# JuliaGaussianProcesses/Stheno.jl

Measured on AMD Instinct MI355X. Metric: logpdf_per_sec, higher is better.
Workload: dtype f64; 1 GPU; single GP, matern52, N=65536, D=8, lengthscale sqrt(D), sigma2=0.1 (BASELINE config 'c5'); N=65536, D=8, kernel=matern52, parallelism=1 GPU

## Files before the change

### stheno.jl_amd/csrc/gemm_nt.hip

```cpp
#include "common.h"
#include "potrf_diag.h"
#include "tilemap.h"
#include "kstep.h"

namespace sgp {

constexpr int KB = 16;

__device__ __forceinline__ bool tile_of_block(long n_tr, long n_tc, long mask_off, long& tr, long& tc) {
  return tile_of_id((long)blockIdx.x, n_tr, n_tc, mask_off, tr, tc);
}

template <bool HANDOFF, bool STAMP = false>
__device__ __forceinline__ bool gemm_nt_dma_tile(const double* A, long lda, const double* B, long ldb, double* C,
                                                 long ldc, long K, double alpha, double beta, long mask_off,
                                                 long n_tr, long n_tc, long c_slice_stride, const double* Cin,
                                                 long ldcin, int klo, double* smem, long& tr, long& tc,
                                                 long long* dbg = nullptr, const TileSkip* sk = nullptr,
                                                 bool keep_first = false) {
  long long st0 = 0, st1 = 0, st2 = 0, stA = 0;
  if (STAMP) st0 = (long long)__builtin_amdgcn_s_memtime();
  constexpr int NJ = 8, WCOLS = 32;
  if (klo == 3) {
    const long sub = mask_off > 1 ? mask_off : 1;
    const long tiles = n_tr * (n_tr + 1) / 2, full = sub > 1 ? tiles / 64 * 64 : tiles;
    const long sl = (long)blockIdx.x & 7;
    long k = (long)blockIdx.x >> 3, q = 0, kk = K;
    if (k >= full) {
      const long e = k - full;
      k = full + e / sub;
      q = e % sub;
      kk = K / sub;
    }
    tr = (long)((sqrt(8.0 * (double)k + 1.0) - 1.0) * 0.5);
    while (tr * (tr + 1) / 2 > k) --tr;
    while ((tr + 1) * (tr + 2) / 2 <= k) ++tr;
    tc = k - tr * (tr + 1) / 2;
    if (tr >= n_tr) return false;
    A += (sl * K + q * kk) * lda;
    B += (sl * K + q * kk) * ldb;
    C += (sl * sub + q) * c_slice_stride;
    K = kk;
  } else {
    if (sk && sk->cmap) {
      const int x = (int)(blockIdx.x & 7), pos = (int)(blockIdx.x >> 3);
      if (pos >= sk->cmap[x]) return false;
      if (!tile_of_id((long)sk->cmap[16 + (long)x * sk->cstride + pos] * 8 + x, n_tr, n_tc, mask_off, tr, tc)) return false;
    } else if (!tile_of_block(n_tr, n_tc, mask_off, tr, tc)) return false;
    A += (long)blockIdx.y * K * lda;
    B += (long)blockIdx.y * K * ldb;
    C += (long)blockIdx.y * c_slice_stride;
  }
  if (sk && sk->nz) {
    if (sk->need0 >= 0) {
      const sz_word* rn = sk->nz + (long)(sk->need0 + tr) * sk->words;
      if (!((rn[tc >> 6] >> (tc & 63)) & 1)) return false;
    }
    const sz_word* ra = sk->nz + (long)(sk->tr0 + tr) * sk->words;
    const sz_word* rb = sk->nz + (long)(sk->tc0 + tc) * sk->words;
    int kmin = -1, kmax = -1;
    for (int q = sk->kt0 >> 6; q <= (sk->kt1 - 1) >> 6; ++q) {
      sz_word m = ra[q] & rb[q];
      if (q == (sk->kt0 >> 6)) m &= ~(sz_word)0 << (sk->kt0 & 63);
      if (q == ((sk->kt1 - 1) >> 6) && (sk->kt1 & 63)) m &= ~(~(sz_word)0 << (sk->kt1 & 63));
      if (m != 0) {
        if (kmin < 0) kmin = q * 64 + (int)__builtin_ctzll(m);
        kmax = q * 64 + 63 - (int)__builtin_clzll(m);
      }
    }
    if (kmin < 0) {
      if (sk->need0 >= 0)
        K = 0;
      else if (!(keep_first && tr == 0 && tc == 0))
        return false;
    } else {
      A += (long)(kmin - sk->kt0) * TILE * lda;
      B += (long)(kmin - sk->kt0) * TILE * ldb;
      K = (long)(kmax - kmin + 1) * TILE;
    }
  }
  if (STAMP) stA = (long long)__builtin_amdgcn_s_memtime();
  const int t = threadIdx.x;
  const int lane = t & 63;
  const int w = t >> 6;
  const int wr = w >> 2, wc = w & 3;
  const int l15 = lane & 15, lq = lane >> 4, l3 = lane & 3;
  const double* Ag = A + tr * TILE;
  const double* Bg = B + tc * TILE;
  double* Cg = C + (tr * TILE + wr * 64 + l15) + (tc * TILE + wc * WCOLS + lq) * ldc;
  const double* Cs = Cin + (tr * TILE + wr * 64 + l15) + (tc * TILE + wc * WCOLS + lq) * ldcin;
  double acc[NJ][4];
  typedef const __attribute__((address_space(1))) void* gptr_t;
  typedef __attribute__((address_space(3))) void* lptr_t;
  const int wu = __builtin_amdgcn_readfirstlane(w);
  const unsigned lds_base = (unsigned)(unsigned long long)(__attribute__((address_space(3))) double*)smem;
  auto dma = [&](long k0, int stage) {
    double* sa = smem + stage * (2 * KB * LDS_LD);
    double* sb = sa + KB * LDS_LD;
#pragma unroll
    for (int i = 0; i < KB / 8; ++i) {
      const int col = wu + 8 * i;
      __builtin_amdgcn_global_load_lds((gptr_t)(Ag + 2 * lane + (k0 + col) * lda), (lptr_t)(sa + col * LDS_LD), 16, 0, 0);
      __builtin_amdgcn_global_load_lds((gptr_t)(Bg + 2 * lane + (k0 + col) * ldb), (lptr_t)(sb + col * LDS_LD), 16, 0, 0);
    }
  };
  long nchunks = K / KB;
  const long cbeg = klo == 1 ? tr * (TILE / KB) : 0;
  if (klo == 2 && (tr + 1) * (TILE / KB) < nchunks) nchunks = (tr + 1) * (TILE / KB);
  auto kof = [&](long c) { return c * KB; };
  if (cbeg < nchunks) dma(kof(cbeg), 0);
  if (beta != 0.0) {
#pragma unroll
    for (int j = 0; j < NJ; ++j)
#pragma unroll
      for (int i = 0; i < 4; ++i) acc[j][i] = Cs[i * 16 + (long)(j * 4) * ldcin];
    const double seed = beta / alpha;
#pragma unroll
    for (int j = 0; j < NJ; ++j)
#pragma unroll
      for (int i = 0; i < 4; ++i) acc[j][i] *= seed;
  } else {
#pragma unroll
    for (int j = 0; j < NJ; ++j)
#pragma unroll
      for (int i = 0; i < 4; ++i) acc[j][i] = 0.0;
  }
  asm volatile("s_waitcnt vmcnt(0)" ::: "memory");
  __builtin_amdgcn_s_barrier();
  if (STAMP) st1 = (long long)__builtin_amdgcn_s_memtime();
  for (long c = cbeg; c < nchunks; ++c) {
    const int stage = (int)(c & 1);
    if (c + 1 < nchunks) dma(kof(c + 1), stage ^ 1);
    const unsigned a_addr = lds_base + (unsigned)((stage * (2 * KB * LDS_LD) + lq * LDS_LD + wr * 64 + l15) * 8);
    const unsigned b_addr = lds_base + (unsigned)((stage * (2 * KB * LDS_LD) + KB * LDS_LD + lq * LDS_LD + wc * WCOLS + l3) * 8);
    {
      double a_r[4], b_c[NJ];
      asm volatile("ds_read_b64 %0, %1 offset:0" : "=v"(a_r[0]) : "v"(a_addr));
      asm volatile("ds_read_b64 %0, %1 offset:128" : "=v"(a_r[1]) : "v"(a_addr));
      asm volatile("ds_read_b64 %0, %1 offset:256" : "=v"(a_r[2]) : "v"(a_addr));
      asm volatile("ds_read_b64 %0, %1 offset:384" : "=v"(a_r[3]) : "v"(a_addr));
      asm volatile("ds_read_b64 %0, %1 offset:0" : "=v"(b_c[0]) : "v"(b_addr));
      asm volatile("ds_read_b64 %0, %1 offset:32" : "=v"(b_c[1]) : "v"(b_addr));
      asm volatile("ds_read_b64 %0, %1 offset:64" : "=v"(b_c[2]) : "v"(b_addr));
      asm volatile("ds_read_b64 %0, %1 offset:96" : "=v"(b_c[3]) : "v"(b_addr));
      asm volatile("ds_read_b64 %0, %1 offset:128" : "=v"(b_c[4]) : "v"(b_addr));
      asm volatile("ds_read_b64 %0, %1 offset:160" : "=v"(b_c[5]) : "v"(b_addr));
      asm volatile("ds_read_b64 %0, %1 offset:192" : "=v"(b_c[6]) : "v"(b_addr));
      asm volatile("ds_read_b64 %0, %1 offset:224" : "=v"(b_c[7]) : "v"(b_addr));
      asm volatile("s_waitcnt lgkmcnt(0)" ::: "memory");
      __builtin_amdgcn_sched_barrier(0);
#pragma unroll
      for (int j = 0; j < NJ; ++j)
#pragma unroll
        for (int i = 0; i < 4; ++i) acc[j][i] = mfma44_f64(b_c[j], a_r[i], acc[j][i]);
    }
    {
      double a_r[4], b_c[NJ];
      asm volatile("ds_read_b64 %0, %1 offset:4608" : "=v"(a_r[0]) : "v"(a_addr));
      asm volatile("ds_read_b64 %0, %1 offset:4736" : "=v"(a_r[1]) : "v"(a_addr));
      asm volatile("ds_read_b64 %0, %1 offset:4864" : "=v"(a_r[2]) : "v"(a_addr));
      asm volatile("ds_read_b64 %0, %1 offset:4992" : "=v"(a_r[3]) : "v"(a_addr));
      asm volatile("ds_read_b64 %0, %1 offset:4608" : "=v"(b_c[0]) : "v"(b_addr));
      asm volatile("ds_read_b64 %0, %1 offset:4640" : "=v"(b_c[1]) : "v"(b_addr));
      asm volatile("ds_read_b64 %0, %1 offset:4672" : "=v"(b_c[2]) : "v"(b_addr));
      asm volatile("ds_read_b64 %0, %1 offset:4704" : "=v"(b_c[3]) : "v"(b_addr));
      asm volatile("ds_read_b64 %0, %1 offset:4736" : "=v"(b_c[4]) : "v"(b_addr));
      asm volatile("ds_read_b64 %0, %1 offset:4768" : "=v"(b_c[5]) : "v"(b_addr));
      asm volatile("ds_read_b64 %0, %1 offset:4800" : "=v"(b_c[6]) : "v"(b_addr));
      asm volatile("ds_read_b64 %0, %1 offset:4832" : "=v"(b_c[7]) : "v"(b_addr));
      asm volatile("s_waitcnt lgkmcnt(0)" ::: "memory");
      __builtin_amdgcn_sched_barrier(0);
#pragma unroll
      for (int j = 0; j < NJ; ++j)
#pragma unroll
        for (int i = 0; i < 4; ++i) acc[j][i] = mfma44_f64(b_c[j], a_r[i], acc[j][i]);
    }
    {
      double a_r[4], b_c[NJ];
      asm volatile("ds_read_b64 %0, %1 offset:9216" : "=v"(a_r[0]) : "v"(a_addr));
      asm volatile("ds_read_b64 %0, %1 offset:9344" : "=v"(a_r[1]) : "v"(a_addr));
      asm volatile("ds_read_b64 %0, %1 offset:9472" : "=v"(a_r[2]) : "v"(a_addr));
      asm volatile("ds_read_b64 %0, %1 offset:9600" : "=v"(a_r[3]) : "v"(a_addr));
      asm volatile("ds_read_b64 %0, %1 offset:9216" : "=v"(b_c[0]) : "v"(b_addr));
      asm volatile("ds_read_b64 %0, %1 offset:9248" : "=v"(b_c[1]) : "v"(b_addr));
      asm volatile("ds_read_b64 %0, %1 offset:9280" : "=v"(b_c[2]) : "v"(b_addr));
      asm volatile("ds_read_b64 %0, %1 offset:9312" : "=v"(b_c[3]) : "v"(b_addr));
      asm volatile("ds_read_b64 %0, %1 offset:9344" : "=v"(b_c[4]) : "v"(b_addr));
      asm volatile("ds_read_b64 %0, %1 offset:9376" : "=v"(b_c[5]) : "v"(b_addr));
      asm volatile("ds_read_b64 %0, %1 offset:9408" : "=v"(b_c[6]) : "v"(b_addr));
      asm volatile("ds_read_b64 %0, %1 offset:9440" : "=v"(b_c[7]) : "v"(b_addr));
      asm volatile("s_waitcnt lgkmcnt(0)" ::: "memory");
      __builtin_amdgcn_sched_barrier(0);
#pragma unroll
      for (int j = 0; j < NJ; ++j)
#pragma unroll
        for (int i = 0; i < 4; ++i) acc[j][i] = mfma44_f64(b_c[j], a_r[i], acc[j][i]);
    }
    {
      double a_r[4], b_c[NJ];
      asm volatile("ds_read_b64 %0, %1 offset:13824" : "=v"(a_r[0]) : "v"(a_addr));
      asm volatile("ds_read_b64 %0, %1 offset:13952" : "=v"(a_r[1]) : "v"(a_addr));
      asm volatile("ds_read_b64 %0, %1 offset:14080" : "=v"(a_r[2]) : "v"(a_addr));
      asm volatile("ds_read_b64 %0, %1 offset:14208" : "=v"(a_r[3]) : "v"(a_addr));
      asm volatile("ds_read_b64 %0, %1 offset:13824" : "=v"(b_c[0]) : "v"(b_addr));
      asm volatile("ds_read_b64 %0, %1 offset:13856" : "=v"(b_c[1]) : "v"(b_addr));
      asm volatile("ds_read_b64 %0, %1 offset:13888" : "=v"(b_c[2]) : "v"(b_addr));
      asm volatile("ds_read_b64 %0, %1 offset:13920" : "=v"(b_c[3]) : "v"(b_addr));
      asm volatile("ds_read_b64 %0, %1 offset:13952" : "=v"(b_c[4]) : "v"(b_addr));
      asm volatile("ds_read_b64 %0, %1 offset:13984" : "=v"(b_c[5]) : "v"(b_addr));
      asm volatile("ds_read_b64 %0, %1 offset:14016" : "=v"(b_c[6]) : "v"(b_addr));
      asm volatile("ds_read_b64 %0, %1 offset:14048" : "=v"(b_c[7]) : "v"(b_addr));
      asm volatile("s_waitcnt lgkmcnt(0)" ::: "memory");
      __builtin_amdgcn_sched_barrier(0);
#pragma unroll
      for (int j = 0; j < NJ; ++j)
#pragma unroll
        for (int i = 0; i < 4; ++i) acc[j][i] = mfma44_f64(b_c[j], a_r[i], acc[j][i]);
    }
    asm volatile("s_waitcnt vmcnt(0) lgkmcnt(0)" ::: "memory");
    __builtin_amdgcn_s_barrier();
  }
  if (STAMP) st2 = (long long)__builtin_amdgcn_s_memtime();
  if (HANDOFF && tr == 0 && tc == 0) {
#pragma unroll
    for (int j = 0; j < NJ; ++j)
#pragma unroll
      for (int i = 0; i < 4; ++i) {
        const int rb = 4 * wr + i, cb = 2 * wc + (j >> 2);
        const int k = 4 * (j & 3) + lq;
        if (rb >= cb) smem[boff(rb, cb) + k * 16 + l15] = (rb > cb || l15 >= k) ? alpha * acc[j][i] : 0.0;
      }
    return true;
  }
#pragma unroll
  for (int j = 0; j < NJ; ++j)
#pragma unroll
    for (int i = 0; i < 4; ++i) Cg[i * 16 + (long)(j * 4) * ldc] = alpha * acc[j][i];
  if (STAMP) {
    asm volatile("s_waitcnt vmcnt(0)" ::: "memory");
    if (threadIdx.x == 0) {
      long long* d = dbg + (long)blockIdx.x * 8;
      d[0] = st0;
      d[1] = st1;
      d[2] = st2;
      d[3] = (long long)__builtin_amdgcn_s_memtime();
      d[4] = (long long)((__builtin_amdgcn_s_getreg(6164) & 15) << 16 | (__builtin_amdgcn_s_getreg(63492) & 0xffff));
      d[5] = tr;
      d[6] = tc;
      d[7] = stA;
    }
  }
  return true;
}

__global__ __launch_bounds__(512, 4) void gemm_nt_dma_stamp_kernel(const double* A, long lda, double* C, long ldc, long K,
                                                                   long n_tr, long n_tc, long long* dbg) {
  __shared__ __attribute__((aligned(16))) double smem[2 * 2 * KB * LDS_LD];
  long tr, tc;
  gemm_nt_dma_tile<false, true>(A, lda, A, lda, C, ldc, K, -1.0, 1.0, 0L, n_tr, n_tc, 0L, C, ldc, 0, smem, tr, tc, dbg);
}

int launch_gemm_nt_stamps(const double* P, long ldp, double* C, long ldc, long M, long Nc, long K, long long* dbg,
                          long* n_ids, hipStream_t s) {
  long n_tr = M / TILE, n_tc = Nc / TILE;
  long per_xcd = tri_ids_per_xcd(tri_shape(n_tr, n_tc, -1));
  *n_ids = per_xcd * 8;
  if (!dbg) return 0;
  hipLaunchKernelGGL(gemm_nt_dma_stamp_kernel, dim3((unsigned)(per_xcd * 8)), dim3(512), 0, s, P, ldp, C, ldc, K, n_tr, n_tc, dbg);
  SGP_HIP(hipGetLastError());
  return 0;
}

template <int TAG>
__global__ __launch_bounds__(512, 4) void gemm_nt_dma_kernel(const double* A, long lda,
                                                             const double* B, long ldb, double* C,
                                                             long ldc, long K, double alpha,
                                                             double beta, long mask_off, long n_tr,
                                                             long n_tc, long c_slice_stride,
                                                             const double* Cin, long ldcin, int klo, TileSkip sk) {
  __shared__ __attribute__((aligned(16))) double smem[2 * 2 * KB * LDS_LD];
  long tr, tc;
  gemm_nt_dma_tile<false>(A, lda, B, ldb, C, ldc, K, alpha, beta, mask_off, n_tr, n_tc, c_slice_stride, Cin, ldcin,
                          klo, smem, tr, tc, nullptr, &sk);
}

template <int TAG, bool HANDOFF>
__global__ __launch_bounds__(512, 4) void gemm_nt_dma_potrf_kernel(const double* A, long lda, const double* B,
                                                                   long ldb, double* C, long ldc, long K,
                                                                   long n_tr, long n_tc, double* invd,
                                                                   double* logdet_slot, int* info, long gcol0,
                                                                   int prio, TileSkip sk) {
  extern __shared__ __attribute__((aligned(16))) double dyn_smem[];
  long tr, tc;
  const bool live = gemm_nt_dma_tile<HANDOFF>(A, lda, B, ldb, C, ldc, K, -1.0, 1.0, 0L, n_tr, n_tc, 0L, C, ldc, 0,
                                              dyn_smem, tr, tc, nullptr, &sk, true);
  if (live && tr == 0 && tc == 0) {
    if (!HANDOFF) {
      __threadfence_block();
    }
    __syncthreads();
    potrf_diag_body<false, double, HANDOFF>(C, ldc, invd, logdet_slot, info, gcol0, prio, nullptr);
  }
}

__global__ __launch_bounds__(512, 4) void gemm_nt_seg_kernel(SegBatch b) {
  __shared__ __attribute__((aligned(16))) double smem[2 * 2 * KB * LDS_LD];
  unsigned id = blockIdx.x;
  if (b.cmap) {
    const int x = (int)(id & 7), pos = (int)(id >> 3);
    if (pos >= b.cmap[x]) return;
    id = (unsigned)b.cmap[16 + (long)x * b.cstride + pos] * 8u + (unsigned)x;
  }
  int d = 0;
  for (int q = 1; q < b.n_dst; ++q)
    if (id >= b.dst[q].id0) d = q;
  d = __builtin_amdgcn_readfirstlane(d);
  const long c0 = b.dst[d].c0;
  const long n_tr = (b.m_tot - c0) / TILE, n_tc = b.dst[d].w / TILE;
  long tr, tc;
  if (!tile_of_id((long)(id - b.dst[d].id0), n_tr, n_tc, 0L, tr, tc)) return;
  const int t = threadIdx.x;
  const int lane = t & 63;
  const int w = t >> 6;
  const int wu = __builtin_amdgcn_readfirstlane(w);
  const int wr = w >> 2, wc = w & 3;
  const int l15 = lane & 15, lq = lane >> 4, l3 = lane & 3;
  const long ldc = b.dst[d].ldc;
  double* Cg = b.dst[d].C + (tr * TILE + wr * 64 + l15) + (tc * TILE + wc * 32 + lq) * ldc;
  typedef const __attribute__((address_space(1))) void* gptr_t;
  typedef __attribute__((address_space(3))) void* lptr_t;
  const unsigned lds_base = (unsigned)(unsigned long long)(__attribute__((address_space(3))) double*)smem;
  int s = b.dst[d].s_first;
  const int s_end = s + b.dst[d].s_count;
  const sz_word* ra = b.nz ? b.nz + (c0 / TILE + tr) * b.nz_words : nullptr;
  const sz_word* rb = b.nz ? b.nz + (c0 / TILE + tc) * b.nz_words : nullptr;
  auto range_of = [&](int q, int& first, int& count) {
    first = 0;
    count = b.src[q].w / KB;
    if (!ra) return;
    const long kc = b.src[q].k0 >= 0 ? b.src[q].k0 : b.src[q].row0;
    const int kt0 = (int)(kc / TILE), kt1 = (int)((kc + b.src[q].w + TILE - 1) / TILE);
    int kmin = -1, kmax = -1;
    for (int k = kt0; k < kt1; ++k)
      if ((((ra[k >> 6] & rb[k >> 6]) >> (k & 63)) & 1) != 0) {
        if (kmin < 0) kmin = k;
        kmax = k;
      }
    if (kmin < 0) {
      count = -1;
    } else if (kc % TILE == 0 && b.src[q].w % TILE == 0) {
      first = (kmin - kt0) * (TILE / KB);
      count = (kmax - kmin + 1) * (TILE / KB);
    }
  };
  unsigned livemask = ~0u;
  long total = 0;
  {
    livemask = 0;
    for (int q = s; q < s_end; ++q) {
      int f, cnt;
      range_of(q, f, cnt);
      if (cnt > 0) {
        livemask |= 1u << q;
        total += cnt;
      }
    }
    if (livemask == 0) return;
    while (!((livemask >> s) & 1)) ++s;
  }
  const double *pa = nullptr, *pb = nullptr;
  long ld = 0;
  int left = 0;
  auto open = [&](int q) {
    const long r0 = c0 - b.src[q].row0;
    ld = b.src[q].ld;
    int f, cnt;
    range_of(q, f, cnt);
    const long skip = (long)f * KB * ld;
    pa = b.src[q].base + r0 + tr * TILE + skip;
    pb = b.src[q].base + r0 + tc * TILE + skip;
    left = cnt;
  };
  auto request = [&](int stage) {
    double* sa = smem + stage * (2 * KB * LDS_LD);
    double* sb = sa + KB * LDS_LD;
#pragma unroll
    for (int i = 0; i < KB / 8; ++i) {
      const int col = wu + 8 * i;
      __builtin_amdgcn_global_load_lds((gptr_t)(pa + 2 * lane + col * ld), (lptr_t)(sa + col * LDS_LD), 16, 0, 0);
      __builtin_amdgcn_global_load_lds((gptr_t)(pb + 2 * lane + col * ld), (lptr_t)(sb + col * LDS_LD), 16, 0, 0);
    }
    pa += KB * ld;
    pb += KB * ld;
    if (--left == 0) {
      ++s;
      while (s < s_end && !((livemask >> s) & 1)) ++s;
      if (s < s_end) open(s);
    }
  };
  double acc[8][4];
  if (total > 0) {
    open(s);
    request(0);
  }
#pragma unroll
  for (int j = 0; j < 8; ++j)
#pragma unroll
    for (int i = 0; i < 4; ++i) acc[j][i] = Cg[i * 16 + (long)(j * 4) * ldc];
#pragma unroll
  for (int j = 0; j < 8; ++j)
#pragma unroll
    for (int i = 0; i < 4; ++i) acc[j][i] *= -1.0;
  asm volatile("s_waitcnt vmcnt(0)" ::: "memory");
  __builtin_amdgcn_s_barrier();
  const unsigned a_off = (unsigned)((lq * LDS_LD + wr * 64 + l15) * 8);
  const unsigned b_off = (unsigned)((KB * LDS_LD + lq * LDS_LD + wc * 32 + l3) * 8);
  for (long c = 0; c < total; ++c) {
    const int stage = (int)(c & 1);
    if (c + 1 < total) request(stage ^ 1);
    const unsigned a_addr = lds_base + (unsigned)(stage * (2 * KB * LDS_LD) * 8) + a_off;
    const unsigned b_addr = lds_base + (unsigned)(stage * (2 * KB * LDS_LD) * 8) + b_off;
    tile_kstep<0>(acc, a_addr, b_addr);
    tile_kstep<1>(acc, a_addr, b_addr);
    tile_kstep<2>(acc, a_addr, b_addr);
    tile_kstep<3>(acc, a_addr, b_addr);
    asm volatile("s_waitcnt vmcnt(0) lgkmcnt(0)" ::: "memory");
    __builtin_amdgcn_s_barrier();
  }
#pragma unroll
  for (int j = 0; j < 8; ++j)
#pragma unroll
    for (int i = 0; i < 4; ++i) Cg[i * 16 + (long)(j * 4) * ldc] = -acc[j][i];
}

__global__ __launch_bounds__(1024) void seg_compact_kernel(SegBatch b, int per_xcd, int* out) {
  __shared__ int s_wave[16];
  __shared__ int s_base;
  const int x = blockIdx.x, t = threadIdx.x, lane = t & 63, w = t >> 6;
  if (t == 0) s_base = 0;
  __syncthreads();
  for (int k0 = 0; k0 < per_xcd; k0 += 1024) {
    const int k = k0 + t;
    bool live = false;
    if (k < per_xcd) {
      const unsigned id = (unsigned)k * 8u + (unsigned)x;
      int d = 0;
      for (int q = 1; q < b.n_dst; ++q)
        if (id >= b.dst[q].id0) d = q;
      const long c0 = b.dst[d].c0;
      long tr, tc;
      if (tile_of_id((long)(id - b.dst[d].id0), (b.m_tot - c0) / TILE, b.dst[d].w / TILE, 0L, tr, tc)) {
        const sz_word* ra = b.nz + (c0 / TILE + tr) * b.nz_words;
        const sz_word* rb = b.nz + (c0 / TILE + tc) * b.nz_words;
        for (int q = b.dst[d].s_first; q < b.dst[d].s_first + b.dst[d].s_count && !live; ++q) {
          const long kc = b.src[q].k0 >= 0 ? b.src[q].k0 : b.src[q].row0;
          const int kt0 = (int)(kc / TILE), kt1 = (int)((kc + b.src[q].w + TILE - 1) / TILE);
          for (int kk = kt0; kk < kt1 && !live; ++kk) live = (((ra[kk >> 6] & rb[kk >> 6]) >> (kk & 63)) & 1) != 0;
        }
      }
    }
    const unsigned long long bal = __ballot(live);
    const int pre = __popcll(bal & ((1ull << lane) - 1ull));
    if (lane == 0) s_wave[w] = __popcll(bal);
    __syncthreads();
    int woff = 0, tot = 0;
    for (int q = 0; q < 16; ++q) {
      if (q < w) woff += s_wave[q];
      tot += s_wave[q];
    }
    const int base = s_base;
    if (live) out[16 + (long)x * per_xcd + base + woff + pre] = k;
    __syncthreads();
    if (t == 0) s_base = base + tot;
    __syncthreads();
  }
  if (t == 0) out[x] = s_base;
}

int launch_gemm_nt_seg(SegBatch& b, hipStream_t s, long* n_ids) {
  if (b.n_dst <= 0) return 0;
  if (b.n_dst > SEG_MAX_DST || b.m_tot % TILE) {
    set_error("gemm_nt_seg: bad batch");
    return -1;
  }
  long ids = 0;
  for (int d = 0; d < b.n_dst; ++d) {
    const SegDst& D = b.dst[d];
    if (D.c0 % TILE || D.w % TILE || D.w <= 0 || D.c0 + D.w > b.m_tot || D.s_first < 0 || D.s_count < 0 ||
        D.s_first + D.s_count > SEG_MAX_SRC) {
      set_error("gemm_nt_seg: bad destination panel");
      return -1;
    }
    for (int q = D.s_first; q < D.s_first + D.s_count; ++q)
      if (b.src[q].w % KB || b.src[q].w <= 0 || b.src[q].row0 > D.c0) {
        set_error("gemm_nt_seg: bad source panel");
        return -1;
      }
    b.dst[d].id0 = (unsigned)ids;
    ids += tile_ids((b.m_tot - D.c0) / TILE, D.w / TILE, 0);
  }
  if (ids >= (1L << 31)) {
    set_error("gemm_nt_seg: too many tiles for one launch");
    return -1;
  }
  if (n_ids) *n_ids = ids;
  const int* map = nullptr;
  if (b.nz && b.map_scratch && ids >= b.map_min_ids && 16 + ids <= b.map_ints) {
    b.cmap = nullptr;
    hipLaunchKernelGGL(seg_compact_kernel, dim3(8), dim3(1024), 0, s, b, (int)(ids / 8), b.map_scratch);
    SGP_HIP(hipGetLastError());
    map = b.map_scratch;
  }
  b.cmap = map;
  b.cstride = (int)(ids / 8);
  hipLaunchKernelGGL(gemm_nt_seg_kernel, dim3((unsigned)ids), dim3(512), 0, s, b);
  SGP_HIP(hipGetLastError());
  return 0;
}

#define SGP_COMPUTE(buf_, NJ_, COL0_)                                            \
  {                                                                              \
    const double* pa = &sA[buf_][wr * 64 + l15];                                 \
    const double* pb = &sB[buf_][(COL0_) + l3];                                  \
    _Pragma("unroll") for (int ks = 0; ks < 4; ++ks) {                           \
      const int kk = ks * 4 + lq;                                                \
      double a_r[4], b_c[NJ_];                                                   \
      _Pragma("unroll") for (int i = 0; i < 4; ++i) a_r[i] = pa[kk * LDS_LD + i * 16]; \
      _Pragma("unroll") for (int j = 0; j < NJ_; ++j) b_c[j] = pb[kk * LDS_LD + j * 4]; \
      _Pragma("unroll") for (int j = 0; j < NJ_; ++j)                            \
          _Pragma("unroll") for (int i = 0; i < 4; ++i)                          \
              acc[j][i] = mfma44_f64(b_c[j], a_r[i], acc[j][i]);                 \
    }                                                                            \
  }

template <bool KCAP>
__global__ __launch_bounds__(512, 4) void gemm_nt_reg_kernel(const double* A, long lda,
                                                             const double* B, long ldb, double* C,
                                                             long ldc, long K, double alpha,
                                                             double beta, long mask_off,
                                                             long kcap_off, long n_tr, long n_tc) {
  constexpr int NJ = 8, WCOLS = 32, NU = 2;
  long tr, tc;
  if (!tile_of_block(n_tr, n_tc, mask_off, tr, tc)) return;
  long Keff = K;
  if (KCAP) {
    long cap = (tc + 1) * TILE + kcap_off;
    if (cap < Keff) Keff = cap;
    if (Keff <= 0) Keff = 0;
  }
  __shared__ __attribute__((aligned(16))) double sA[2][KB * LDS_LD];
  __shared__ __attribute__((aligned(16))) double sB[2][KB * LDS_LD];
  const int t = threadIdx.x;
  const int lane = t & 63;
  const int w = t >> 6;
  const int wr = w >> 2, wc = w & 3;
  const int l15 = lane & 15, lq = lane >> 4, l3 = lane & 3;
  const double* Ag = A + tr * TILE;
  const double* Bg = B + tc * TILE;
  const int scol = t >> 6;
  const int srow = 2 * (t & 63);
  double2 ra[NU], rb[NU];
  double* Cg = C + (tr * TILE + wr * 64 + l15) + (tc * TILE + wc * WCOLS + lq) * ldc;
  double acc[NJ][4];
  if (beta != 0.0) {
    const double seed = beta / alpha;
#pragma unroll
    for (int j = 0; j < NJ; ++j)
#pragma unroll
      for (int i = 0; i < 4; ++i) acc[j][i] = Cg[i * 16 + (long)(j * 4) * ldc];
#pragma unroll
    for (int j = 0; j < NJ; ++j)
#pragma unroll
      for (int i = 0; i < 4; ++i) acc[j][i] *= seed;
  } else {
#pragma unroll
    for (int j = 0; j < NJ; ++j)
#pragma unroll
      for (int i = 0; i < 4; ++i) acc[j][i] = 0.0;
  }
#define SGP_GLOAD(k0_)                                                           \
  _Pragma("unroll") for (int i = 0; i < NU; ++i) {                               \
    long col = (k0_) + scol + 8 * i;                                             \
    ra[i] = *reinterpret_cast<const double2*>(Ag + srow + col * lda);            \
    rb[i] = *reinterpret_cast<const double2*>(Bg + srow + col * ldb);            \
  }
#define SGP_SSTORE(buf_)                                                         \
  _Pragma("unroll") for (int i = 0; i < NU; ++i) {                               \
    int col = scol + 8 * i;                                                      \
    *reinterpret_cast<double2*>(&sA[buf_][col * LDS_LD + srow]) = ra[i];         \
    *reinterpret_cast<double2*>(&sB[buf_][col * LDS_LD + srow]) = rb[i];         \
  }
  if (Keff > 0) {
    SGP_GLOAD(0);
    SGP_SSTORE(0);
    __syncthreads();
    int buf = 0;
    for (long k0 = KB; k0 < Keff; k0 += KB) {
      SGP_GLOAD(k0);
      SGP_COMPUTE(buf, NJ, wc * WCOLS);
      SGP_SSTORE(buf ^ 1);
      __syncthreads();
      buf ^= 1;
    }
    SGP_COMPUTE(buf, NJ, wc * WCOLS);
  }
#undef SGP_GLOAD
#undef SGP_SSTORE
#pragma unroll
  for (int j = 0; j < NJ; ++j)
#pragma unroll
    for (int i = 0; i < 4; ++i) Cg[i * 16 + (long)(j * 4) * ldc] = alpha * acc[j][i];
}

namespace {
struct GemmStructure {
  const char* base = nullptr;
  long elem = 8;
  long ld = 0;
  const sz_word* nz = nullptr;
  int words = 0;
  int* scratch = nullptr;
  long scratch_ints = 0;
  long tile0 = 0;
  long ncols = 0;
  hipStream_t stream2 = nullptr;
  int* scratch2 = nullptr;
};
thread_local GemmStructure g_st;
TileSkip skip_for_bytes(const void* P, long ldp, const void* C, long ldc, long K, long elem) {
  TileSkip sk;
  if (!g_st.nz || ldp != g_st.ld || ldc != g_st.ld || elem != g_st.elem) return sk;
  const long oc = ((const char*)C - g_st.base) / elem, op = ((const char*)P - g_st.base) / elem;
  if ((const char*)C < g_st.base || (const char*)P < g_st.base || oc >= g_st.ld * g_st.ncols || op >= g_st.ld * g_st.ncols) return sk;
  const long cr = oc % g_st.ld, cc = oc / g_st.ld, pr = op % g_st.ld, pc = op / g_st.ld;
  if (cr != cc || pr != cr || cr % TILE || pc % TILE || K % TILE || pc + K > cc) return sk;
  sk.nz = g_st.nz;
  sk.words = g_st.words;
  sk.tr0 = sk.tc0 = (int)(cr / TILE + g_st.tile0);
  sk.kt0 = (int)(pc / TILE + g_st.tile0);
  sk.kt1 = sk.kt0 + (int)(K / TILE);
  return sk;
}
TileSkip skip_for(const double* P, long ldp, const double* C, long ldc, long K) { return skip_for_bytes(P, ldp, C, ldc, K, 8); }
StripSkip strip_skip_bytes(const void* X, long ldx, long elem) {
  StripSkip sk;
  if (!g_st.nz || ldx != g_st.ld || elem != g_st.elem || (const char*)X < g_st.base) return sk;
  const long ox = ((const char*)X - g_st.base) / elem;
  if (ox >= g_st.ld * g_st.ncols) return sk;
  const long xr = ox % g_st.ld, xc = ox / g_st.ld;
  if (xr % TILE || xc % TILE || xr <= xc) return sk;
  sk.nz = g_st.nz;
  sk.words = g_st.words;
  sk.tr0 = (int)(xr / TILE + g_st.tile0);
  sk.kt = (int)(xc / TILE + g_st.tile0);
  return sk;
}
}
void gemm_set_structure(const double* base, long ld, const sz_word* d_nz, int words, long ncols, int* scratch,
                        long scratch_ints, long tile0, hipStream_t stream2, int* scratch2) {
  g_st.base = (const char*)base;
  g_st.elem = 8;
  g_st.ld = ld;
  g_st.nz = d_nz;
  g_st.words = words;
  g_st.scratch = scratch;
  g_st.scratch_ints = scratch_ints;
  g_st.tile0 = tile0;
  g_st.ncols = ncols;
  g_st.stream2 = stream2;
  g_st.scratch2 = scratch2;
}
void gemm_set_structure_f32(const float* base, long ld, const sz_word* d_nz, int words, long ncols) {
  gemm_set_structure(nullptr, ld, d_nz, words, ncols);
  g_st.base = (const char*)base;
  g_st.elem = 4;
}
TileSkip gemm_skip_for_f32(const float* P, long ldp, const float* C, long ldc, long K) { return skip_for_bytes(P, ldp, C, ldc, K, 4); }
StripSkip strip_skip_for_f32(const float* X, long ldx) { return strip_skip_bytes(X, ldx, 4); }
StripSkip strip_skip_for(const double* X, long ldx) { return strip_skip_bytes(X, ldx, 8); }

__global__ __launch_bounds__(1024) void tile_compact_kernel(TileSkip sk, long n_tr, long n_tc, int per_xcd, int* out,
                                                            int keep_first) {
  __shared__ int s_wave[16];
  __shared__ int s_base;
  const int x = blockIdx.x, t = threadIdx.x, lane = t & 63, w = t >> 6;
  if (t == 0) s_base = 0;
  __syncthreads();
  for (int k0 = 0; k0 < per_xcd; k0 += 1024) {
    const int k = k0 + t;
    bool live = false;
    long tr, tc;
    if (k < per_xcd && tile_of_id((long)k * 8 + x, n_tr, n_tc, 0L, tr, tc)) {
      const sz_word* ra = sk.nz + (long)(sk.tr0 + tr) * sk.words;
      const sz_word* rb = sk.nz + (long)(sk.tc0 + tc) * sk.words;
      for (int q = sk.kt0 >> 6; q <= (sk.kt1 - 1) >> 6; ++q) {
        sz_word m = ra[q] & rb[q];
        if (q == (sk.kt0 >> 6)) m &= ~(sz_word)0 << (sk.kt0 & 63);
        if (q == ((sk.kt1 - 1) >> 6) && (sk.kt1 & 63)) m &= ~(~(sz_word)0 << (sk.kt1 & 63));
        live = live || m != 0;
      }
      live = live || (keep_first && tr == 0 && tc == 0);
    }
    const unsigned long long bal = __ballot(live);
    const int pre = __popcll(bal & ((1ull << lane) - 1ull));
    if (lane == 0) s_wave[w] = __popcll(bal);
    __syncthreads();
    int woff = 0, tot = 0;
    for (int q = 0; q < 16; ++q) {
      if (q < w) woff += s_wave[q];
      tot += s_wave[q];
    }
    const int base = s_base;
    if (live) out[16 + (long)x * per_xcd + base + woff + pre] = k;
    __syncthreads();
    if (t == 0) s_base = base + tot;
    __syncthreads();
  }
  if (t == 0) out[x] = s_base;
}
static int maybe_compact(TileSkip& sk, long n_tr, long n_tc, long per_xcd, int keep_first, hipStream_t s) {
  int* map = (g_st.scratch2 && s == g_st.stream2) ? g_st.scratch2 : g_st.scratch;
  if (!sk.nz || !map || per_xcd * 8 < 4096 || 16 + per_xcd * 8 > g_st.scratch_ints) return 0;
  hipLaunchKernelGGL(tile_compact_kernel, dim3(8), dim3(1024), 0, s, sk, n_tr, n_tc, (int)per_xcd, map, keep_first);
  SGP_HIP(hipGetLastError());
  sk.cmap = map;
  sk.cstride = (int)per_xcd;
  return 0;
}

int launch_gemm_nt(const double* A, long lda, const double* B, long ldb, double* C, long ldc,
                   long M, long Nc, long K, double alpha, double beta, long mask_off,
                   int kcap_mode, long kcap_off, hipStream_t s) {
  constexpr long REG_BASELINE = -(1L << 50);
  if (M <= 0 || Nc <= 0) return 0;
  if (M % TILE || Nc % TILE || K % KB) {
    set_error("gemm_nt: M, Nc must be multiples of 128 and K of 16");
    return -1;
  }
  long n_tr = M / TILE, n_tc = Nc / TILE;
  long groups = ((n_tr + 7) / 8 + 7) / 8;
  long per_xcd = (mask_off == 0) ? tri_ids_per_xcd(tri_shape(n_tr, n_tc, -1)) : groups * 8 * n_tc;
  dim3 grid((unsigned)(per_xcd * 8));
  if (kcap_mode)
    hipLaunchKernelGGL((gemm_nt_reg_kernel<true>), grid, dim3(512), 0, s, A, lda, B, ldb, C, ldc, K, alpha,
                       beta, mask_off, kcap_off, n_tr, n_tc);
  else if (kcap_off == REG_BASELINE)
    hipLaunchKernelGGL((gemm_nt_reg_kernel<false>), grid, dim3(512), 0, s, A, lda, B, ldb, C, ldc, K, alpha,
                       beta, mask_off, 0L, n_tr, n_tc);
  else
    hipLaunchKernelGGL(gemm_nt_dma_kernel<0>, grid, dim3(512), 0, s, A, lda, B, ldb, C, ldc, K, alpha, beta,
                       mask_off, n_tr, n_tc, 0L, (const double*)C, ldc, 0,
                       (A == B && mask_off == 0 && alpha == -1.0 && beta == 1.0) ? skip_for(A, lda, C, ldc, K) : TileSkip());
  SGP_HIP(hipGetLastError());
  return 0;
}

int launch_gemm_nt_update(const double* P, long ldp, double* C, long ldc, long M, long Nc, long K, hipStream_t s) {
  if (M <= 0 || Nc <= 0) return 0;
  if (M % TILE || Nc % TILE || K % KB) {
    set_error("gemm_nt_update: M, Nc must be multiples of 128 and K of 16");
    return -1;
  }
  long n_tr = M / TILE, n_tc = Nc / TILE;
  long per_xcd = tri_ids_per_xcd(tri_shape(n_tr, n_tc, -1));
  TileSkip sk = skip_for(P, ldp, C, ldc, K);
  if (int rc = maybe_compact(sk, n_tr, n_tc, per_xcd, 0, s)) return rc;
  hipLaunchKernelGGL(gemm_nt_dma_kernel<1>, dim3((unsigned)(per_xcd * 8)), dim3(512), 0, s, P, ldp, P, ldp, C, ldc, K,
                     -1.0, 1.0, 0L, n_tr, n_tc, 0L, (const double*)C, ldc, 0, sk);
  SGP_HIP(hipGetLastError());
  return 0;
}

template <int TAG, bool HANDOFF>
static int launch_potrf_variant(unsigned grid, const double* P, long ldp, double* C, long ldc, long K, long n_tr,
                                long n_tc, double* d_invd, double* d_logdet_slot, int* d_info, long gcol0,
                                hipStream_t s) {
  SGP_LDS_ATTR_ONCE((gemm_nt_dma_potrf_kernel<TAG, HANDOFF>), PD_LDS);
  TileSkip sk = skip_for(P, ldp, C, ldc, K);
  if (int rc = maybe_compact(sk, n_tr, n_tc, (long)grid / 8, 1, s)) return rc;
  hipLaunchKernelGGL((gemm_nt_dma_potrf_kernel<TAG, HANDOFF>), dim3(grid), dim3(512), PD_LDS, s, P, ldp, P, ldp, C, ldc,
                     K, n_tr, n_tc, d_invd, d_logdet_slot, d_info, gcol0, panel_prio(), sk);
  SGP_HIP(hipGetLastError());
  return 0;
}

int launch_gemm_nt_potrf(const double* P, long ldp, double* C, long ldc, long M, long Nc, long K, int outer,
                         int handoff, double* d_invd, double* d_logdet_slot, int* d_info, long gcol0,
                         hipStream_t s) {
  if (M <= 0 || Nc <= 0) return 0;
  if (M % TILE || Nc % TILE || K % KB) {
    set_error("gemm_nt_potrf: M, Nc must be multiples of 128 and K of 16");
    return -1;
  }
  long n_tr = M / TILE, n_tc = Nc / TILE;
  long per_xcd = tri_ids_per_xcd(tri_shape(n_tr, n_tc, -1));
  const unsigned grid = (unsigned)(per_xcd * 8);
  if (outer)
    return handoff ? launch_potrf_variant<1, true>(grid, P, ldp, C, ldc, K, n_tr, n_tc, d_invd, d_logdet_slot, d_info, gcol0, s)
                   : launch_potrf_variant<1, false>(grid, P, ldp, C, ldc, K, n_tr, n_tc, d_invd, d_logdet_slot, d_info, gcol0, s);
  return handoff ? launch_potrf_variant<0, true>(grid, P, ldp, C, ldc, K, n_tr, n_tc, d_invd, d_logdet_slot, d_info, gcol0, s)
                 : launch_potrf_variant<0, false>(grid, P, ldp, C, ldc, K, n_tr, n_tc, d_invd, d_logdet_slot, d_info, gcol0, s);
}

int launch_gemm_nt_cin(const double* A, long lda, const double* B, long ldb, const double* Cin, long ldcin,
                       double* C, long ldc, long M, long Nc, long K, double alpha, double beta,
                       hipStream_t s) {
  if (M <= 0 || Nc <= 0) return 0;
  if (M % TILE || Nc % TILE || K % KB) {
    set_error("gemm_nt_cin: M, Nc must be multiples of 128 and K of 16");
    return -1;
  }
  long n_tr = M / TILE, n_tc = Nc / TILE;
  long groups = ((n_tr + 7) / 8 + 7) / 8;
  dim3 grid((unsigned)(groups * 8 * n_tc * 8));
  hipLaunchKernelGGL(gemm_nt_dma_kernel<0>, grid, dim3(512), 0, s, A, lda, B, ldb, C, ldc, K, alpha, beta,
                     -(1L << 40), n_tr, n_tc, 0L, Cin, ldcin, 0, TileSkip());
  SGP_HIP(hipGetLastError());
  return 0;
}

int launch_gemm_nt_uut(const double* X, long ldx, double* C, long ldc, long n, hipStream_t s, const TileSkip* sk) {
  if (n <= 0) return 0;
  if (n % TILE) {
    set_error("gemm_nt_uut: n must be a multiple of 128");
    return -1;
  }
  long n_t = n / TILE;
  long per_xcd = tri_ids_per_xcd(tri_shape(n_t, n_t, -1));
  if (sk && sk->nz) {
    TileSkip k2 = *sk;
    k2.kt0 = 0;
    k2.kt1 = (int)n_t;
    k2.cmap = nullptr;
    hipLaunchKernelGGL(gemm_nt_dma_kernel<0>, dim3((unsigned)(per_xcd * 8)), dim3(512), 0, s, X, ldx, X, ldx, C, ldc, n,
                       1.0, 0.0, 0L, n_t, n_t, 0L, (const double*)C, ldc, 0, k2);
  } else
    hipLaunchKernelGGL(gemm_nt_dma_kernel<0>, dim3((unsigned)(per_xcd * 8)), dim3(512), 0, s, X, ldx, X, ldx, C, ldc, n,
                       1.0, 0.0, 0L, n_t, n_t, 0L, (const double*)C, ldc, 1, TileSkip());
  SGP_HIP(hipGetLastError());
  return 0;
}

struct UutBatch {
  const double* X[DF_MAX_BATCH];
  double* C[DF_MAX_BATCH];
};
__global__ __launch_bounds__(512, 4) void gemm_nt_uut_batch_kernel(UutBatch b, long ldx, long ldc, long n, long n_t) {
  __shared__ __attribute__((aligned(16))) double smem[2 * 2 * KB * LDS_LD];
  const double* X = b.X[blockIdx.z];
  double* C = b.C[blockIdx.z];
  const TileSkip none;
  long tr, tc;
  gemm_nt_dma_tile<false>(X, ldx, X, ldx, C, ldc, n, 1.0, 0.0, 0L, n_t, n_t, 0L, (const double*)C, ldc, 1, smem, tr, tc,
                          nullptr, &none);
}
int launch_gemm_nt_uut_batch(const double* const* X, long ldx, double* const* C, long ldc, long n, int nb, hipStream_t s) {
  if (n <= 0 || nb <= 0) return 0;
  if (n % TILE || nb > DF_MAX_BATCH) {
    set_error("gemm_nt_uut_batch: n must be a multiple of 128 and the batch at most DF_MAX_BATCH");
    return -1;
  }
  UutBatch b;
  for (int i = 0; i < DF_MAX_BATCH; ++i) {
    b.X[i] = i < nb ? X[i] : nullptr;
    b.C[i] = i < nb ? C[i] : nullptr;
  }
  const long n_t = n / TILE;
  const long per_xcd = tri_ids_per_xcd(tri_shape(n_t, n_t, -1));
  hipLaunchKernelGGL(gemm_nt_uut_batch_kernel, dim3((unsigned)(per_xcd * 8), 1, (unsigned)nb), dim3(512), 0, s, b, ldx, ldc,
                     n, n_t);
  SGP_HIP(hipGetLastError());
  return 0;
}

int launch_gemm_nt_lz_k(const double* L, long ldl, const double* Zt, long ldz, double* C, long ldc, long n,
                        long ns, long K, double beta, hipStream_t s) {
  if (n <= 0 || ns <= 0 || K <= 0) return 0;
  if (n % TILE || ns % TILE || K % TILE) {
    set_error("gemm_nt_lz: n, ns, K must be multiples of 128");
    return -1;
  }
  long n_tr = n / TILE, n_tc = ns / TILE;
  long groups = ((n_tr + 7) / 8 + 7) / 8;
  hipLaunchKernelGGL(gemm_nt_dma_kernel<0>, dim3((unsigned)(groups * 8 * n_tc * 8)), dim3(512), 0, s, L, ldl, Zt, ldz, C,
                     ldc, K, 1.0, beta, -(1L << 40), n_tr, n_tc, 0L, (const double*)C, ldc, 2, TileSkip());
  SGP_HIP(hipGetLastError());
  return 0;
}
int launch_gemm_nt_lz(const double* L, long ldl, const double* Zt, long ldz, double* C, long ldc, long n,
                      long ns, double beta, hipStream_t s) {
  return launch_gemm_nt_lz_k(L, ldl, Zt, ldz, C, ldc, n, ns, n, beta, s);
}

long splitk_sub(long M, long K) {
  const long n_t = M / TILE, tiles = n_t * (n_t + 1) / 2, left = tiles % 64;
  if (left == 0 || tiles < 64 || 64 % left) return 1;
  const long sub = 64 / left;
  if (sub < 2 || sub > 8 || K % (8 * sub * KB)) return 1;
  return sub;
}
long splitk_slabs(long M, long K, int nsplit) { return nsplit == 8 ? 8 * splitk_sub(M, K) : nsplit; }

int launch_gemm_nt_splitk(const double* A, long lda, const double* B, long ldb, double* Cpart, long ldc,
                          long M, long Nc, long K, int nsplit, long part_stride, int lower_only,
                          hipStream_t s) {
  if (M % TILE || Nc % TILE || nsplit < 1 || K % (KB * (long)nsplit)) {
    set_error("gemm_nt_splitk: bad sizes");
    return -1;
  }
  long n_tr = M / TILE, n_tc = Nc / TILE;
  if (lower_only && nsplit == 8 && M == Nc) {
    const long tiles = n_tr * (n_tr + 1) / 2;
    const long sub = splitk_sub(M, K);
    const long full = sub > 1 ? tiles / 64 * 64 : tiles;
    const long ids = full + (tiles - full) * sub;
    hipLaunchKernelGGL(gemm_nt_dma_kernel<0>, dim3((unsigned)(ids * 8)), dim3(512), 0, s, A, lda, B, ldb, Cpart, ldc,
                       K / nsplit, 1.0, 0.0, sub, n_tr, n_tc, part_stride, (const double*)Cpart, ldc, 3, TileSkip());
    SGP_HIP(hipGetLastError());
    return 0;
  }
  long groups = ((n_tr + 7) / 8 + 7) / 8;
  long mask_off = lower_only ? 0 : -(1L << 40);
  long per_xcd = lower_only ? tri_ids_per_xcd(tri_shape(n_tr, n_tc, -1)) : groups * 8 * n_tc;
  dim3 grid((unsigned)(per_xcd * 8), (unsigned)nsplit);
  hipLaunchKernelGGL(gemm_nt_dma_kernel<0>, grid, dim3(512), 0, s, A, lda, B, ldb, Cpart, ldc, K / nsplit, 1.0,
                     0.0, mask_off, n_tr, n_tc, part_stride, (const double*)Cpart, ldc, 0, TileSkip());
  SGP_HIP(hipGetLastError());
  return 0;
}

__global__ void splitk_reduce_kernel(const double* part, long part_stride, int nsplit, double* C,
                                     long ldc, long M, long Nc, double alpha, double beta,
                                     int lower_only, int sub, long full) {
  long idx = (long)blockIdx.x * blockDim.x + threadIdx.x;
  if (idx >= M * Nc) return;
  long r = idx % M, c = idx / M;
  const long tr = r / TILE, tc = c / TILE;
  if (lower_only && tr < tc) return;
  double s = 0.0;
  if (sub > 1) {
    const bool whole = tr * (tr + 1) / 2 + tc < full;
    const int step = whole ? sub : 1;
    for (int k = 0; k < nsplit * sub; k += step) s += part[k * part_stride + r + c * ldc];
  } else {
    for (int k = 0; k < nsplit; ++k) s += part[k * part_stride + r + c * ldc];
  }
  double* p = C + r + c * ldc;
  double old = (beta == 0.0) ? 0.0 : beta * (*p);
  *p = old + alpha * s;
}

int launch_splitk_reduce(const double* part, long part_stride, int nsplit, double* C, long ldc, long M,
                         long Nc, double alpha, double beta, int lower_only, hipStream_t s, long K) {
  long tot = M * Nc;
  const long sub = (K > 0 && lower_only && nsplit == 8 && M == Nc) ? splitk_sub(M, K) : 1;
  const long n_t = M / TILE, tiles = n_t * (n_t + 1) / 2;
  hipLaunchKernelGGL(splitk_reduce_kernel, dim3((unsigned)((tot + 255) / 256)), dim3(256), 0, s, part,
                     part_stride, nsplit, C, ldc, M, Nc, alpha, beta, lower_only, (int)sub, tiles / 64 * 64);
  SGP_HIP(hipGetLastError());
  return 0;
}

}
```

Measured before the change: 0.6900 logpdf/s.

## Remap GEMM thread ownership for 128-bit LDS reads and buffer-load DMA

Rewrites the thread-to-output mapping so each lane owns 4 consecutive rows and 8 consecutive columns. LDS operand fetches can then use ds_read_b128 instead of scalar ds_read_b64, roughly halving LDS read instructions per k-step. Global-to-LDS copies switch from global_load_lds to buffer_load_lds with a new LDS pitch of 130, and C loads and stores become 16-byte vector accesses. The new layout risks LDS bank conflicts under the changed pitch and needs the handoff path's diagonal masking to be remapped correctly, which the code does.

```diff
diff --git a/stheno.jl_amd/csrc/gemm_nt.hip b/stheno.jl_amd/csrc/gemm_nt.hip
--- a/stheno.jl_amd/csrc/gemm_nt.hip
+++ b/stheno.jl_amd/csrc/gemm_nt.hip
@@ -6,6 +6,38 @@
 namespace sgp {
 
 constexpr int KB = 16;
+
+constexpr int DMA_LD = 130;
+constexpr int DMA_STAGE = 2 * KB * DMA_LD;
+typedef double d2 __attribute__((ext_vector_type(2)));
+typedef double d2u __attribute__((ext_vector_type(2), aligned(8)));
+
+__device__ __forceinline__ void column_dma(const double* col, double* lds, unsigned voff) {
+#if defined(__HIP_DEVICE_COMPILE__)
+  __builtin_amdgcn_raw_ptr_buffer_load_lds(__builtin_amdgcn_make_buffer_rsrc((void*)col, (short)0, TILE * 8, 0x00020000),
+                                           (__attribute__((address_space(3))) void*)lds, 16, voff, 0, 0, 0);
+#endif
+}
+
+template <int KS>
+__device__ __forceinline__ void wide_kstep(double (&acc)[8][4], unsigned a_addr, unsigned b_addr) {
+  constexpr int O = KS * 4 * DMA_LD * 8;
+  d2 a01, a23, b01, b23, b45, b67;
+  asm volatile("ds_read_b128 %0, %1 offset:%2" : "=v"(a01) : "v"(a_addr), "i"(O));
+  asm volatile("ds_read_b128 %0, %1 offset:%2" : "=v"(a23) : "v"(a_addr), "i"(O + 16));
+  asm volatile("ds_read_b128 %0, %1 offset:%2" : "=v"(b01) : "v"(b_addr), "i"(O));
+  asm volatile("ds_read_b128 %0, %1 offset:%2" : "=v"(b23) : "v"(b_addr), "i"(O + 16));
+  asm volatile("ds_read_b128 %0, %1 offset:%2" : "=v"(b45) : "v"(b_addr), "i"(O + 32));
+  asm volatile("ds_read_b128 %0, %1 offset:%2" : "=v"(b67) : "v"(b_addr), "i"(O + 48));
+  asm volatile("s_waitcnt lgkmcnt(0)" ::: "memory");
+  __builtin_amdgcn_sched_barrier(0);
+  const double a_r[4] = {a01.x, a01.y, a23.x, a23.y};
+  const double b_c[8] = {b01.x, b01.y, b23.x, b23.y, b45.x, b45.y, b67.x, b67.y};
+#pragma unroll
+  for (int j = 0; j < 8; ++j)
+#pragma unroll
+    for (int i = 0; i < 4; ++i) acc[j][i] = mfma44_f64(b_c[j], a_r[i], acc[j][i]);
+}
 
 __device__ __forceinline__ bool tile_of_block(long n_tr, long n_tc, long mask_off, long& tr, long& tc) {
   return tile_of_id((long)blockIdx.x, n_tr, n_tc, mask_off, tr, tc);
@@ -87,21 +119,20 @@
   const int l15 = lane & 15, lq = lane >> 4, l3 = lane & 3;
   const double* Ag = A + tr * TILE;
   const double* Bg = B + tc * TILE;
-  double* Cg = C + (tr * TILE + wr * 64 + l15) + (tc * TILE + wc * WCOLS + lq) * ldc;
-  const double* Cs = Cin + (tr * TILE + wr * 64 + l15) + (tc * TILE + wc * WCOLS + lq) * ldcin;
+  double* Cg = C + (tr * TILE + wr * 64 + 4 * l15) + (tc * TILE + wc * WCOLS + 8 * lq) * ldc;
+  const double* Cs = Cin + (tr * TILE + wr * 64 + 4 * l15) + (tc * TILE + wc * WCOLS + 8 * lq) * ldcin;
   double acc[NJ][4];
-  typedef const __attribute__((address_space(1))) void* gptr_t;
-  typedef __attribute__((address_space(3))) void* lptr_t;
   const int wu = __builtin_amdgcn_readfirstlane(w);
   const unsigned lds_base = (unsigned)(unsigned long long)(__attribute__((address_space(3))) double*)smem;
+  const unsigned voff = (unsigned)lane * 16u;
   auto dma = [&](long k0, int stage) {
-    double* sa = smem + stage * (2 * KB * LDS_LD);
-    double* sb = sa + KB * LDS_LD;
+    double* sa = smem + stage * DMA_STAGE;
+    double* sb = sa + KB * DMA_LD;
 #pragma unroll
     for (int i = 0; i < KB / 8; ++i) {
       const int col = wu + 8 * i;
-      __builtin_amdgcn_global_load_lds((gptr_t)(Ag + 2 * lane + (k0 + col) * lda), (lptr_t)(sa + col * LDS_LD), 16, 0, 0);
-      __builtin_amdgcn_global_load_lds((gptr_t)(Bg + 2 * lane + (k0 + col) * ldb), (lptr_t)(sb + col * LDS_LD), 16, 0, 0);
+      column_dma(Ag + (k0 + col) * lda, sa + col * DMA_LD, voff);
+      column_dma(Bg + (k0 + col) * ldb, sb + col * DMA_LD, voff);
     }
   };
   long nchunks = K / KB;
@@ -111,9 +142,14 @@
   if (cbeg < nchunks) dma(kof(cbeg), 0);
   if (beta != 0.0) {
 #pragma unroll
-    for (int j = 0; j < NJ; ++j)
-#pragma unroll
-      for (int i = 0; i < 4; ++i) acc[j][i] = Cs[i * 16 + (long)(j * 4) * ldcin];
+    for (int j = 0; j < NJ; ++j) {
+      const d2u* p = (const d2u*)(Cs + (long)j * ldcin);
+      const d2u lo = p[0], hi = p[1];
+      acc[j][0] = lo.x;
+      acc[j][1] = lo.y;
+      acc[j][2] = hi.x;
+      acc[j][3] = hi.y;
+    }
     const double seed = beta / alpha;
 #pragma unroll
     for (int j = 0; j < NJ; ++j)
@@ -131,111 +167,35 @@
   for (long c = cbeg; c < nchunks; ++c) {
     const int stage = (int)(c & 1);
     if (c + 1 < nchunks) dma(kof(c + 1), stage ^ 1);
-    const unsigned a_addr = lds_base + (unsigned)((stage * (2 * KB * LDS_LD) + lq * LDS_LD + wr * 64 + l15) * 8);
-    const unsigned b_addr = lds_base + (unsigned)((stage * (2 * KB * LDS_LD) + KB * LDS_LD + lq * LDS_LD + wc * WCOLS + l3) * 8);
-    {
-      double a_r[4], b_c[NJ];
-      asm volatile("ds_read_b64 %0, %1 offset:0" : "=v"(a_r[0]) : "v"(a_addr));
-      asm volatile("ds_read_b64 %0, %1 offset:128" : "=v"(a_r[1]) : "v"(a_addr));
-      asm volatile("ds_read_b64 %0, %1 offset:256" : "=v"(a_r[2]) : "v"(a_addr));
-      asm volatile("ds_read_b64 %0, %1 offset:384" : "=v"(a_r[3]) : "v"(a_addr));
-      asm volatile("ds_read_b64 %0, %1 offset:0" : "=v"(b_c[0]) : "v"(b_addr));
-      asm volatile("ds_read_b64 %0, %1 offset:32" : "=v"(b_c[1]) : "v"(b_addr));
-      asm volatile("ds_read_b64 %0, %1 offset:64" : "=v"(b_c[2]) : "v"(b_addr));
-      asm volatile("ds_read_b64 %0, %1 offset:96" : "=v"(b_c[3]) : "v"(b_addr));
-      asm volatile("ds_read_b64 %0, %1 offset:128" : "=v"(b_c[4]) : "v"(b_addr));
-      asm volatile("ds_read_b64 %0, %1 offset:160" : "=v"(b_c[5]) : "v"(b_addr));
-      asm volatile("ds_read_b64 %0, %1 offset:192" : "=v"(b_c[6]) : "v"(b_addr));
-      asm volatile("ds_read_b64 %0, %1 offset:224" : "=v"(b_c[7]) : "v"(b_addr));
-      asm volatile("s_waitcnt lgkmcnt(0)" ::: "memory");
-      __builtin_amdgcn_sched_barrier(0);
-#pragma unroll
-      for (int j = 0; j < NJ; ++j)
-#pragma unroll
-        for (int i = 0; i < 4; ++i) acc[j][i] = mfma44_f64(b_c[j], a_r[i], acc[j][i]);
-    }
-    {
-      double a_r[4], b_c[NJ];
-      asm volatile("ds_read_b64 %0, %1 offset:4608" : "=v"(a_r[0]) : "v"(a_addr));
-      asm volatile("ds_read_b64 %0, %1 offset:4736" : "=v"(a_r[1]) : "v"(a_addr));
-      asm volatile("ds_read_b64 %0, %1 offset:4864" : "=v"(a_r[2]) : "v"(a_addr));
-      asm volatile("ds_read_b64 %0, %1 offset:4992" : "=v"(a_r[3]) : "v"(a_addr));
-      asm volatile("ds_read_b64 %0, %1 offset:4608" : "=v"(b_c[0]) : "v"(b_addr));
-      asm volatile("ds_read_b64 %0, %1 offset:4640" : "=v"(b_c[1]) : "v"(b_addr));
-      asm volatile("ds_read_b64 %0, %1 offset:4672" : "=v"(b_c[2]) : "v"(b_addr));
-      asm volatile("ds_read_b64 %0, %1 offset:4704" : "=v"(b_c[3]) : "v"(b_addr));
-      asm volatile("ds_read_b64 %0, %1 offset:4736" : "=v"(b_c[4]) : "v"(b_addr));
-      asm volatile("ds_read_b64 %0, %1 offset:4768" : "=v"(b_c[5]) : "v"(b_addr));
-      asm volatile("ds_read_b64 %0, %1 offset:4800" : "=v"(b_c[6]) : "v"(b_addr));
-      asm volatile("ds_read_b64 %0, %1 offset:4832" : "=v"(b_c[7]) : "v"(b_addr));
-      asm volatile("s_waitcnt lgkmcnt(0)" ::: "memory");
-      __builtin_amdgcn_sched_barrier(0);
-#pragma unroll
-      for (int j = 0; j < NJ; ++j)
-#pragma unroll
-        for (int i = 0; i < 4; ++i) acc[j][i] = mfma44_f64(b_c[j], a_r[i], acc[j][i]);
-    }
-    {
-      double a_r[4], b_c[NJ];
-      asm volatile("ds_read_b64 %0, %1 offset:9216" : "=v"(a_r[0]) : "v"(a_addr));
-      asm volatile("ds_read_b64 %0, %1 offset:9344" : "=v"(a_r[1]) : "v"(a_addr));
-      asm volatile("ds_read_b64 %0, %1 offset:9472" : "=v"(a_r[2]) : "v"(a_addr));
-      asm volatile("ds_read_b64 %0, %1 offset:9600" : "=v"(a_r[3]) : "v"(a_addr));
-      asm volatile("ds_read_b64 %0, %1 offset:9216" : "=v"(b_c[0]) : "v"(b_addr));
-      asm volatile("ds_read_b64 %0, %1 offset:9248" : "=v"(b_c[1]) : "v"(b_addr));
-      asm volatile("ds_read_b64 %0, %1 offset:9280" : "=v"(b_c[2]) : "v"(b_addr));
-      asm volatile("ds_read_b64 %0, %1 offset:9312" : "=v"(b_c[3]) : "v"(b_addr));
-      asm volatile("ds_read_b64 %0, %1 offset:9344" : "=v"(b_c[4]) : "v"(b_addr));
-      asm volatile("ds_read_b64 %0, %1 offset:9376" : "=v"(b_c[5]) : "v"(b_addr));
-      asm volatile("ds_read_b64 %0, %1 offset:9408" : "=v"(b_c[6]) : "v"(b_addr));
-      asm volatile("ds_read_b64 %0, %1 offset:9440" : "=v"(b_c[7]) : "v"(b_addr));
-      asm volatile("s_waitcnt lgkmcnt(0)" ::: "memory");
-      __builtin_amdgcn_sched_barrier(0);
-#pragma unroll
-      for (int j = 0; j < NJ; ++j)
-#pragma unroll
-        for (int i = 0; i < 4; ++i) acc[j][i] = mfma44_f64(b_c[j], a_r[i], acc[j][i]);
-    }
-    {
-      double a_r[4], b_c[NJ];
-      asm volatile("ds_read_b64 %0, %1 offset:13824" : "=v"(a_r[0]) : "v"(a_addr));
-      asm volatile("ds_read_b64 %0, %1 offset:13952" : "=v"(a_r[1]) : "v"(a_addr));
-      asm volatile("ds_read_b64 %0, %1 offset:14080" : "=v"(a_r[2]) : "v"(a_addr));
-      asm volatile("ds_read_b64 %0, %1 offset:14208" : "=v"(a_r[3]) : "v"(a_addr));
-      asm volatile("ds_read_b64 %0, %1 offset:13824" : "=v"(b_c[0]) : "v"(b_addr));
-      asm volatile("ds_read_b64 %0, %1 offset:13856" : "=v"(b_c[1]) : "v"(b_addr));
-      asm volatile("ds_read_b64 %0, %1 offset:13888" : "=v"(b_c[2]) : "v"(b_addr));
-      asm volatile("ds_read_b64 %0, %1 offset:13920" : "=v"(b_c[3]) : "v"(b_addr));
-      asm volatile("ds_read_b64 %0, %1 offset:13952" : "=v"(b_c[4]) : "v"(b_addr));
-      asm volatile("ds_read_b64 %0, %1 offset:13984" : "=v"(b_c[5]) : "v"(b_addr));
-      asm volatile("ds_read_b64 %0, %1 offset:14016" : "=v"(b_c[6]) : "v"(b_addr));
-      asm volatile("ds_read_b64 %0, %1 offset:14048" : "=v"(b_c[7]) : "v"(b_addr));
-      asm volatile("s_waitcnt lgkmcnt(0)" ::: "memory");
-      __builtin_amdgcn_sched_barrier(0);
-#pragma unroll
-      for (int j = 0; j < NJ; ++j)
-#pragma unroll
-        for (int i = 0; i < 4; ++i) acc[j][i] = mfma44_f64(b_c[j], a_r[i], acc[j][i]);
-    }
+    const unsigned a_addr = lds_base + (unsigned)((stage * DMA_STAGE + lq * DMA_LD + wr * 64 + 4 * l15) * 8);
+    const unsigned b_addr = lds_base + (unsigned)((stage * DMA_STAGE + KB * DMA_LD + lq * DMA_LD + wc * WCOLS + 8 * l3) * 8);
+    wide_kstep<0>(acc, a_addr, b_addr);
+    wide_kstep<1>(acc, a_addr, b_addr);
+    wide_kstep<2>(acc, a_addr, b_addr);
+    wide_kstep<3>(acc, a_addr, b_addr);
     asm volatile("s_waitcnt vmcnt(0) lgkmcnt(0)" ::: "memory");
     __builtin_amdgcn_s_barrier();
   }
   if (STAMP) st2 = (long long)__builtin_amdgcn_s_memtime();
   if (HANDOFF && tr == 0 && tc == 0) {
-#pragma unroll
-    for (int j = 0; j < NJ; ++j)
-#pragma unroll
-      for (int i = 0; i < 4; ++i) {
-        const int rb = 4 * wr + i, cb = 2 * wc + (j >> 2);
-        const int k = 4 * (j & 3) + lq;
-        if (rb >= cb) smem[boff(rb, cb) + k * 16 + l15] = (rb > cb || l15 >= k) ? alpha * acc[j][i] : 0.0;
-      }
+    const int rb = 4 * wr + (l15 >> 2), cb = 2 * wc + (lq >> 1);
+    if (rb >= cb) {
+#pragma unroll
+      for (int j = 0; j < NJ; ++j)
+#pragma unroll
+        for (int i = 0; i < 4; ++i) {
+          const int m = 4 * (l15 & 3) + i, k = 8 * (lq & 1) + j;
+          smem[boff(rb, cb) + k * 16 + m] = (rb > cb || m >= k) ? alpha * acc[j][i] : 0.0;
+        }
+    }
     return true;
   }
 #pragma unroll
-  for (int j = 0; j < NJ; ++j)
-#pragma unroll
-    for (int i = 0; i < 4; ++i) Cg[i * 16 + (long)(j * 4) * ldc] = alpha * acc[j][i];
+  for (int j = 0; j < NJ; ++j) {
+    d2u* p = (d2u*)(Cg + (long)j * ldc);
+    p[0] = d2u{alpha * acc[j][0], alpha * acc[j][1]};
+    p[1] = d2u{alpha * acc[j][2], alpha * acc[j][3]};
+  }
   if (STAMP) {
     asm volatile("s_waitcnt vmcnt(0)" ::: "memory");
     if (threadIdx.x == 0) {
@@ -255,7 +215,7 @@
 
 __global__ __launch_bounds__(512, 4) void gemm_nt_dma_stamp_kernel(const double* A, long lda, double* C, long ldc, long K,
                                                                    long n_tr, long n_tc, long long* dbg) {
-  __shared__ __attribute__((aligned(16))) double smem[2 * 2 * KB * LDS_LD];
+  __shared__ __attribute__((aligned(16))) double smem[2 * DMA_STAGE];
   long tr, tc;
   gemm_nt_dma_tile<false, true>(A, lda, A, lda, C, ldc, K, -1.0, 1.0, 0L, n_tr, n_tc, 0L, C, ldc, 0, smem, tr, tc, dbg);
 }
@@ -278,7 +238,7 @@
                                                              double beta, long mask_off, long n_tr,
                                                              long n_tc, long c_slice_stride,
                                                              const double* Cin, long ldcin, int klo, TileSkip sk) {
-  __shared__ __attribute__((aligned(16))) double smem[2 * 2 * KB * LDS_LD];
+  __shared__ __attribute__((aligned(16))) double smem[2 * DMA_STAGE];
   long tr, tc;
   gemm_nt_dma_tile<false>(A, lda, B, ldb, C, ldc, K, alpha, beta, mask_off, n_tr, n_tc, c_slice_stride, Cin, ldcin,
                           klo, smem, tr, tc, nullptr, &sk);
@@ -846,7 +806,7 @@
   double* C[DF_MAX_BATCH];
 };
 __global__ __launch_bounds__(512, 4) void gemm_nt_uut_batch_kernel(UutBatch b, long ldx, long ldc, long n, long n_t) {
-  __shared__ __attribute__((aligned(16))) double smem[2 * 2 * KB * LDS_LD];
+  __shared__ __attribute__((aligned(16))) double smem[2 * DMA_STAGE];
   const double* X = b.X[blockIdx.z];
   double* C = b.C[blockIdx.z];
   const TileSkip none;
```

Result: no change. 0.6955 logpdf/s (median of 6 runs) (+0.8%).
